# HuaiLeiTang/slam_ros

Measured on NVIDIA B200. Metric: EKF predict+update steps/s at N landmarks, higher is better.
Workload: dtype f64

## Files before the change

### slam_ros_b200/csrc/ekf_api.cu

```cuda
#include "../../include/ekf.h"
#include "ekf_internal.h"

#include <cuda.h>
#include <dlfcn.h>
#include <math.h>
#include <stdio.h>
#include <stdlib.h>
#include <string.h>
#include <vector>

namespace {
typedef struct ncclComm* ncclComm_t;
typedef struct { char internal[128]; } ncclUniqueId;
struct NcclApi {
  void* handle;
  int (*GetUniqueId)(ncclUniqueId*);
  int (*CommInitRank)(ncclComm_t*, int, ncclUniqueId, int);
  int (*CommDestroy)(ncclComm_t);
  int (*AllReduce)(const void*, void*, size_t, int, int, ncclComm_t, cudaStream_t);
  const char* (*GetErrorString)(int);
};
const int kNcclFloat64 = 8, kNcclSum = 0;

NcclApi* nccl_api() {
// ... 72 lines not shown
  double* xchg;
  void* peer_map[8];
  EkfPeers peers;
  int peers_mapped;
  int peers_ok;
  int poisoned;
  double* d_stage; size_t stage_elems;
  double* d_partials; double* d_out3;
  char err[256];
};

namespace {

#define CU(call)                                                                              \
  do {                                                                                        \
    cudaError_t e_ = (call);                                                                  \
    if (e_ != cudaSuccess) {                                                                  \
      snprintf(ctx->err, sizeof ctx->err, "%s:%d %.120s: %s", "ekf_api.cu", __LINE__, #call, cudaGetErrorString(e_)); \
      return EKF_ECUDA;                                                                       \
    }                                                                                         \
  } while (0)

#define NOT_POISONED(ctx)                                                                                          \
  do {                                                                                                             \
    if ((ctx)->poisoned) {                                                                                         \
      snprintf((ctx)->err, sizeof (ctx)->err, "a cross-GPU exchange timed out earlier (EKF_ENCCL): re-upload the state with ekf_upload"); \
      return EKF_ESTATE;                                                                                           \
    }                                                                                                              \
  } while (0)

const size_t kStageElems = (size_t)8 << 20;
const int kOverlapMinN = 6000;
static int line_sms_env() { static int v = -2; if (v == -2) { const char* e = getenv("EKF_LINE_SMS"); v = e ? atoi(e) : -1; if (v < 1 || v > 64) v = -1; } return v; }
static int line_sms_for(int world, int cap, int m) {
  const int e = line_sms_env();
  if (e > 0) return e;
  if (world >= 4) return 28;
  const int need = (cap + 511) / 512;
  return (world == 1 && m > 8 && need > 20 && need <= 28) ? need : 20;
}

double* in_u(ekf_ctx* c) { return c->d_in; }
double* in_x(ekf_ctx* c) { return c->d_in + 3; }
double* in_z(ekf_ctx* c) { return c->d_in + 6; }
double* in_R(ekf_ctx* c) { return c->d_in + 6 + 2 * (size_t)c->max_lines; }

void use_tables(ekf_ctx* ctx, int t) {
  ctx->b.jbest = ctx->tab[t].jbest; ctx->b.jout = ctx->tab[t].jout; ctx->b.pidx = ctx->tab[t].pidx;
  ctx->b.eidx = ctx->tab[t].eidx; ctx->b.ext = ctx->tab[t].ext; ctx->b.ext_cs = ctx->tab[t].ext_cs;
}

int free_line_tables(ekf_ctx* ctx) {
  for (int t = 0; t < 2; ++t) {
    cudaFree(ctx->tab[t].jbest); cudaFree(ctx->tab[t].jout); cudaFree(ctx->tab[t].pidx); cudaFree(ctx->tab[t].eidx);
    cudaFree(ctx->tab[t].ext); cudaFree(ctx->tab[t].ext_cs);
    memset(&ctx->tab[t], 0, sizeof ctx->tab[t]);
  }
  cudaFree(ctx->d_in);
  cudaFreeHost(ctx->h_in); cudaFreeHost(ctx->h_jout);
  ctx->b.jbest = ctx->b.jout = ctx->b.pidx = ctx->b.eidx = ctx->b.ext = 0; ctx->b.ext_cs = 0; ctx->d_in = 0;
  ctx->h_in = 0; ctx->h_jout = 0;
  return 0;
}

int drain(ekf_ctx* ctx);
int close_group(ekf_ctx* ctx);

int ensure_lines(ekf_ctx* ctx, int m) {
  if (m <= ctx->max_lines) return EKF_OK;
  if (ctx->scan_open && ctx->cursor > 0) {
    snprintf(ctx->err, sizeof ctx->err, "scan has more than %d lines; raise it by calling ekf_scan once with m lines", ctx->max_lines);
    return EKF_EINVAL;
// ... 176 lines not shown
  cudaEvent_t e0 = 0, e1 = 0;
  if (ctx->prof) {
    if (ctx->ev_used + 2 > ctx->ev.size())
      for (int i = 0; i < 64; ++i) { cudaEvent_t e; CU(cudaEventCreate(&e)); ctx->ev.push_back(e); }
    e0 = ctx->ev[ctx->ev_used]; e1 = ctx->ev[ctx->ev_used + 1];
    CU(cudaEventRecord(e0, ctx->wstream));
  }
  CU(ekf_launch_sweep_tma(ctx->g, bt, &ctx->tmap2[tgt], ctx->have_tmap8 ? &ctx->tmap8[tgt] : 0, &ctx->tmapK[0], &ctx->tmapK[1], ctx->Pbuf[tgt ^ 1], slot0, &ctx->d_view[par], ctx->d_counters + 16,
                          ctx->sweep_shape, nterms, L_ub, ctx->num_sms - line_sms, ctx->wstream,
                          &ctx->tmap2[tgt ^ 1], ctx->have_tmap8 ? &ctx->tmap8[tgt ^ 1] : 0));
  { const int per_pass = ekf_sweep_terms_per_pass(ctx->sweep_shape, nterms); ctx->launches += (nterms + per_pass - 1) / per_pass; }
  if (ctx->prof) {
    CU(cudaEventRecord(e1, ctx->wstream));
    ctx->ev_used += 2;
    ctx->ev_bytes.push_back((double)nterms);
  }
  CU(cudaEventRecord(ctx->evF[par], ctx->wstream));
  ctx->evF_used[par] = 1;
  ctx->rd = tgt; ctx->pg_valid = 1; ctx->pg_slot0 = slot0;
  ctx->par ^= 1;
  ctx->b.P = ctx->Pbuf[ctx->rd];
  return EKF_OK;
}

int close_group(ekf_ctx* ctx) {
  if (!ctx->grp_open) return EKF_OK;
  ctx->grp_open = 0;
  return hand_off_sweep(ctx, ctx->grp_terms, ctx->L_ub, ctx->grp_line_sms);
}

int enqueue_scan_overlapped(ekf_ctx* ctx, const double* d_u, const double* d_x_t0, int m, const double* d_z, const double* d_R) {
  const bool chunked = ctx->chunk_lines > 0 && m > ctx->chunk_above && ctx->g.world == 1;
  const int chunk = chunked ? ctx->chunk_lines : m;
  const int line_sms = line_sms_for(ctx->g.world, ctx->g.cap, m);
  const bool groupable = ctx->grp_budget > 0 && !chunked && ctx->g.world == 1;
  const bool joins = groupable && ctx->grp_open && ctx->grp_terms + m <= ctx->grp_budget && line_sms == ctx->grp_line_sms;
  if (!joins) { int rc = close_group(ctx); if (rc) return rc; }
  const int grp_terms = joins ? ctx->grp_terms + m : m;
  const bool stays_open = groupable && grp_terms + m <= ctx->grp_budget;
  if (line_sms > ctx->last_line_sms && ctx->pg_valid && ctx->evF_used[ctx->par ^ 1])
    CU(cudaStreamWaitEvent(ctx->stream, ctx->evF[ctx->par ^ 1], 0));
  ctx->last_line_sms = line_sms;
  use_tables(ctx, ctx->tabpar);
  ctx->tabpar ^= 1;
  long long lub = (long long)ctx->L_ub + m;
  const int L_after_ub = (int)(lub > ctx->g.cap ? ctx->g.cap : lub);
  { int rc = line_event(ctx); if (rc) return rc; }
  for (int line0 = 0; line0 < m; line0 += chunk) {
    const int line1 = line0 + chunk < m ? line0 + chunk : m;
    const bool first = line0 == 0, last = line1 == m;
    const int par = ctx->par;
    if (ctx->evF_used[par]) CU(cudaStreamWaitEvent(ctx->stream, ctx->evF[par], 0));
    const int slot0 = par * ctx->group;
    EkfBuffers b = ctx->b;
    b.P = ctx->Pbuf[ctx->rd];
    const int* carry = joins ? &ctx->d_view[par].cnt : 0;
    const bool fuse = first && ekf_scan_lines_fuses_predict(ctx->peers_ok ? &ctx->peers : 0) && !ctx->no_fuse;
    if (first && !fuse) { CU(ekf_launch_predict(ctx->g, b, d_u, d_x_t0, m, ctx->L_ub, ctx->stream, carry)); ctx->launches++; }
    CU(ekf_launch_scan_lines(ctx->g, b, d_z, d_R, line0, line1, line_sms, 1, slot0, ctx->pg_slot0,
                             ctx->pg_valid ? &ctx->d_view[par ^ 1].cnt : 0, ctx->peers_ok ? &ctx->peers : 0, ctx->L_ub, ctx->stream,
                             fuse ? d_u : 0, fuse ? d_x_t0 : 0, m, fuse ? carry : 0));
    ctx->launches++;
    const int tgt = ctx->pg_valid ? (ctx->rd ^ 1) : ctx->rd;
    EkfBuffers bt = ctx->b;
    bt.P = ctx->Pbuf[tgt];
    if (last) {
      if (joins && ctx->grp_may_reset && ctx->pg_valid && ctx->evF_used[par ^ 1])
// ... 823 lines not shown
```

### slam_ros_b200/csrc/ekf_internal.h

```cpp
#ifndef EKF_INTERNAL_H
#define EKF_INTERNAL_H

#include <cuda_runtime.h>
#include <limits.h>

#define EKF_TILE 64
#define EKF_LD_ALIGN 256
#define EKF_NO_MATCH INT_MAX
#define EKF_STICKY_CAPACITY 1
#define EKF_STICKY_SINGULAR 2
#define EKF_STICKY_XCHG 4

struct EkfDevState {
  double pose[3];
  double x_pre[3];
  double v[2];
  double S[4];
  int L;
  int epoch;
  int sticky;
  int n_added;
  int resets;
  int pbase;
  int np;
  int xseq;
  int L0;
};

struct EkfScanView { int cnt; int L; int pad[2]; };

struct EkfPeers { double* xchg[8]; int world, rank; };

struct EkfGeom {
  int cap;
  int n;
  int ld;
  int rank, world;
  double gate, enc_noise;
  int headroom;
  double gate_d2max;
};

struct EkfBuffers {
  EkfDevState* st;
  double* y;
  double* top;
  double* diag;
  double* P;
  int* matched;
  double2* Kp;
  double2* KSp;
  double* gates;
  double* colA;
  double* colB;
  int* jbest;
  int* jout;
  int* pidx;
  int* eidx;
  int* ext;
// ... 60 lines not shown
```

### slam_ros_b200/csrc/ekf_kernels.cu

```cuda
#include "ekf_internal.h"
#include "ekf_device.cuh"
#include <stdlib.h>
#include <string.h>
#include <cuda.h>
#include <cooperative_groups.h>
namespace cg = cooperative_groups;

#define EKF_BLOCK 256

namespace {

__device__ __forceinline__ int owner_of_row(const EkfGeom& g, int r) { return (r / EKF_TILE) % g.world; }
__device__ __forceinline__ size_t local_row(const EkfGeom& g, int r) {
  return (size_t)((r / EKF_TILE) / g.world) * EKF_TILE + (size_t)(r % EKF_TILE);
}
__device__ __forceinline__ bool is_hot(int r, int q) {
  return r <= 2 || q == r || (q == r + 1 && (r & 1));
}
__device__ __forceinline__ double hot_value(const EkfGeom& g, const EkfBuffers& b, int r, int q) {
  if (r <= 2) return b.top[(size_t)r * g.ld + q];
  const int j = (r - 3) >> 1;
  if (r & 1) return b.diag[4 * j + (q - r)];
  return b.diag[4 * j + 2];
}
// ... 318 lines not shown
      for (int t = 0; t < 8; ++t) if (i0 + t < npt) {
        d.pa = sub_rank2(d.pa, d.v[t], s_ka[i0 + t]);
        d.pb = sub_rank2(d.pb, d.v[t], s_kb[i0 + t]);
      }
    }
  } else if (d.kind == 2) {
    for (int i0 = 0; i0 < npt; i0 += 8) {
      if (i0 > 0) {
#pragma unroll
        for (int t = 0; t < 8; ++t) if (i0 + t < npt) d.v[t] = b.Kp[(size_t)pl.slot(i0 + t) * g.ld + r];
      }
#pragma unroll
      for (int t = 0; t < 8; ++t) if (i0 + t < npt) {
        d.pa = sub_rank2(d.pa, s_ksa[i0 + t], d.v[t]);
        d.pb = sub_rank2(d.pb, s_ksb[i0 + t], d.v[t]);
      }
    }
  }
}
__device__ __forceinline__ void gain_row_emit(const EkfGeom& g, const EkfBuffers& b, const Gate& G, int r, int out_slot,
                                              const GainRow& d) {
  double2 Kr, KSr;
  gain_row(G, d.p0, d.p1, d.p2, d.pa, d.pb, Kr, KSr);
  b.Kp[(size_t)out_slot * g.ld + r] = Kr;
  b.KSp[(size_t)out_slot * g.ld + r] = KSr;
}

__device__ __forceinline__ double* xchg_col(const EkfPeers& pe, const EkfGeom& g, int p, int par, int which) {
  return pe.xchg[p] + ((size_t)(2 * par + which)) * g.ld;
}
__device__ __forceinline__ unsigned long long* xchg_flags(const EkfPeers& pe, const EkfGeom& g, int p) {
  return reinterpret_cast<unsigned long long*>(pe.xchg[p] + (size_t)4 * g.ld);
}
__device__ __forceinline__ unsigned long long ld_acquire_sys(const unsigned long long* p) {
  unsigned long long v;
  asm volatile("ld.acquire.sys.global.u64 %0, [%1];" : "=l"(v) : "l"(p) : "memory");
  return v;
}
__device__ __forceinline__ void st_relaxed_sys(unsigned long long* p, unsigned long long v) {
  asm volatile("st.relaxed.sys.global.u64 [%0], %1;" ::"l"(p), "l"(v) : "memory");
}
__device__ __forceinline__ void xgpu_exchange_barrier(const EkfPeers& pe, const EkfGeom& g, unsigned long long epoch, int* sticky) {
  __threadfence_system();
  for (int p = 0; p < pe.world; ++p) st_relaxed_sys(xchg_flags(pe, g, p) + pe.rank, epoch);
  const unsigned long long* mine = xchg_flags(pe, g, pe.rank);
  for (int q = 0; q < pe.world; ++q) {
    long long spins = 0;
    while (ld_acquire_sys(mine + q) < epoch) {
      if (++spins > 40000000LL) { atomicOr(sticky, EKF_STICKY_XCHG); break; }
    }
  }
}

#ifdef EKF_LINE_TIMING
__device__ unsigned long long g_line_ts[64 * 16];
__device__ __forceinline__ unsigned long long gtimer() { unsigned long long t; asm volatile("mov.u64 %0, %%globaltimer;" : "=l"(t)); return t; }
#define TS(slot) do { if (gtid == 0 && line - line0 < 64) g_line_ts[(line - line0) * 16 + (slot)] = gtimer(); } while (0)
#else
#define TS(slot) do { } while (0)
#endif

template <int FL_THREADS, bool COOP, bool SHARD>
__global__ void __launch_bounds__(FL_THREADS, FL_THREADS == 256 ? 3 : 1) k_scan_lines(EkfGeom g, EkfBuffers b, const double* __restrict__ z,
                                                              const double* __restrict__ R, int line0, int line1,
                                                              int own_slot0, int prev_slot0, const int* __restrict__ prev_cnt_ptr,
                                                              EkfPeers pe) {
  __shared__ int s_min[FL_THREADS / 32];
  __shared__ double2 s_ka[FL_MAXP], s_kb[FL_MAXP], s_ksa[FL_MAXP], s_ksb[FL_MAXP];
  const int prev_cnt = prev_cnt_ptr ? *prev_cnt_ptr : 0;
  EkfDevState* st = b.st;
  const int gtid = blockIdx.x * blockDim.x + threadIdx.x;
  const int gstride = gridDim.x * blockDim.x;
  auto group_sync = [] () {
    if (COOP) cg::this_grid().sync(); else cg::this_cluster().sync();
  };
  const int L = st->L, nl = 3 + 2 * L, epoch = st->epoch, pbase = st->pbase;
  int nm = b.pidx[line0];
  int ne = b.eidx[line0];
  const int xseq0 = SHARD ? st->xseq : 0;
  int xdone = 0;
  double A[3][3], xp[3];
  load_rr(g, b.top, A);
  xp[0] = st->x_pre[0]; xp[1] = st->x_pre[1]; xp[2] = st->x_pre[2];
  bool have_prev = false;
  int np_prev = 0;
  double pv0 = 0.0, pv1 = 0.0;
  double pS[4] = {0, 0, 0, 0};
  for (int line = line0; line <= line1; ++line) {
    const bool gating = line < line1;
    if (!gating && !have_prev) break;
    TS(0);
    double Rl[4] = {0, 0, 0, 0}, z0 = 0, z1 = 0;
// ... 171 lines not shown
    nm += 1;
    pv0 = G.v[0]; pv1 = G.v[1];
    for (int t = 0; t < 4; ++t) pS[t] = G.S[t];
  }
  if (SHARD && gtid == 0) st->xseq = xseq0 + xdone;
}

struct HotLm { double t0a, t0b, t1a, t1b, t2a, t2b, daa, dab, dbb, ya, yb; int mt; };
__device__ __forceinline__ void hot_load(const EkfGeom& g, const EkfBuffers& b, int j, HotLm& h) {
  const int a = 3 + 2 * j;
  h.t0a = b.top[a]; h.t0b = b.top[a + 1];
  h.t1a = b.top[(size_t)g.ld + a]; h.t1b = b.top[(size_t)g.ld + a + 1];
  h.t2a = b.top[(size_t)2 * g.ld + a]; h.t2b = b.top[(size_t)2 * g.ld + a + 1];
  h.daa = b.diag[4 * j]; h.dab = b.diag[4 * j + 1]; h.dbb = b.diag[4 * j + 2];
  h.ya = b.y[a]; h.yb = b.y[a + 1];
  h.mt = b.matched[j];
}
__device__ __forceinline__ void hot_store(const EkfGeom& g, const EkfBuffers& b, int j, const HotLm& h) {
  const int a = 3 + 2 * j;
  b.top[a] = h.t0a; b.top[a + 1] = h.t0b;
  b.top[(size_t)g.ld + a] = h.t1a; b.top[(size_t)g.ld + a + 1] = h.t1b;
  b.top[(size_t)2 * g.ld + a] = h.t2a; b.top[(size_t)2 * g.ld + a + 1] = h.t2b;
  b.diag[4 * j] = h.daa; b.diag[4 * j + 1] = h.dab; b.diag[4 * j + 2] = h.dbb;
  b.y[a] = h.ya; b.y[a + 1] = h.yb;
}

template <int FL_THREADS, bool COOP, bool CACHED>
__global__ void __launch_bounds__(FL_THREADS, 1) k_scan_lines2(EkfGeom g, EkfBuffers b, const double* __restrict__ z,
                                                               const double* __restrict__ R, int line0, int line1,
                                                               int own_slot0, int prev_slot0, const int* __restrict__ prev_cnt_ptr,
                                                               const double* __restrict__ pred_u, const double* __restrict__ pred_x, int pred_m,
                                                               const int* __restrict__ pred_carry) {
  __shared__ int s_min[FL_THREADS / 32];
  __shared__ double2 s_ka[FL_MAXP], s_kb[FL_MAXP], s_ksa[FL_MAXP], s_ksb[FL_MAXP];
  const int prev_cnt = prev_cnt_ptr ? *prev_cnt_ptr : 0;
  EkfDevState* st = b.st;
  const int gtid = blockIdx.x * blockDim.x + threadIdx.x;
  const int gstride = gridDim.x * blockDim.x;
  const int scribe = gstride - 1;
  auto group_sync = [] () {
    if (COOP) cg::this_grid().sync(); else cg::this_cluster().sync();
  };
  if (pred_u) {
    predict_body(g, b, pred_u, pred_x, pred_m, gtid, gstride, pred_carry);
    __threadfence();
    group_sync();
  }
  const int L = st->L, epoch = st->epoch, pbase = st->pbase;
  int nm = b.pidx[line0];
  int ne = b.eidx[line0];
  double A[3][3], xp[3];
  load_rr(g, b.top, A);
  xp[0] = st->x_pre[0]; xp[1] = st->x_pre[1]; xp[2] = st->x_pre[2];
  constexpr bool cached = CACHED;
  HotLm h;
  if (cached && gtid < L) hot_load(g, b, gtid, h);
  PendingList pl;
  pl.prev_cnt = prev_cnt; pl.prev_slot0 = prev_slot0; pl.own_slot0 = own_slot0;
  for (int line = line0; line < line1; ++line) {
    TS(0);
    const double Rl[4] = {R[4 * line], R[4 * line + 1], R[4 * line + 2], R[4 * line + 3]};
    const double z0 = z[2 * line], z1 = z[2 * line + 1];
    int cand = EKF_NO_MATCH;
    for (int j = gtid; j < L; j += gstride) {
      if (!cached) hot_load(g, b, j, h);
      if (cand == EKF_NO_MATCH && h.mt != epoch) {
        double Cm[5][5];
        for (int r = 0; r < 3; ++r) for (int q = 0; q < 3; ++q) Cm[r][q] = A[r][q];
        Cm[0][3] = Cm[3][0] = h.t0a; Cm[0][4] = Cm[4][0] = h.t0b;
        Cm[1][3] = Cm[3][1] = h.t1a; Cm[1][4] = Cm[4][1] = h.t1b;
        Cm[2][3] = Cm[3][2] = h.t2a; Cm[2][4] = Cm[4][2] = h.t2b;
        Cm[3][3] = h.daa; Cm[3][4] = Cm[4][3] = h.dab; Cm[4][4] = h.dbb;
        Gate G;
        gate_from_block(Cm, h.ya, h.yb, xp, z0, z1, Rl, G);
        if (G.singular) atomicOr(&st->sticky, EKF_STICKY_SINGULAR);
        else if (!gate_rejects_d2(G.d2, g.gate_d2max)) {
          cand = j;
          double* rec = b.gates + (size_t)GATE_REC * j;
          gate_store(rec, G);
          rec[14] = h.t0a; rec[15] = h.t0b; rec[16] = h.t1a; rec[17] = h.t1b; rec[18] = h.t2a; rec[19] = h.t2b;
        }
      }
    }
    TS(1);
    cand = __reduce_min_sync(0xffffffffu, cand);
    if ((threadIdx.x & 31) == 0) s_min[threadIdx.x >> 5] = cand;
    __syncthreads();
    if (threadIdx.x < 32) {
      int v = (threadIdx.x < FL_THREADS / 32) ? s_min[threadIdx.x] : EKF_NO_MATCH;
      v = __reduce_min_sync(0xffffffffu, v);
      if (threadIdx.x == 0 && v != EKF_NO_MATCH) atomicMin(&b.jbest[line], v);
    }
    TS(2);
    group_sync();
    TS(3);
    const int jw = b.jbest[line];
    const int np = nm - pbase;
    if (jw != EKF_NO_MATCH) TS(8);
    if (jw == EKF_NO_MATCH) {
      if (gtid == scribe) { b.ext[ne] = line; b.eidx[line + 1] = ne + 1; b.pidx[line + 1] = nm; b.jout[line] = -1; }
      ne += 1;
      continue;
    }
    const int aw = 3 + 2 * jw, bw = aw + 1;
    const double* rec = b.gates + (size_t)GATE_REC * jw;
    Gate G;
    gate_load(rec, G);
    TS(9);
    const double wt[3][2] = {{rec[14], rec[15]}, {rec[16], rec[17]}, {rec[18], rec[19]}};
    const int npt = prev_cnt + np;
    for (int i = threadIdx.x; i < npt; i += blockDim.x) {
      const int slot = pl.slot(i);
      s_ka[i] = b.Kp[(size_t)slot * g.ld + aw]; s_kb[i] = b.Kp[(size_t)slot * g.ld + bw];
      s_ksa[i] = b.KSp[(size_t)slot * g.ld + aw]; s_ksb[i] = b.KSp[(size_t)slot * g.ld + bw];
    }
    const int out_slot = own_slot0 + np;
    double2 kk[3], ks[3];
#pragma unroll
    for (int r = 0; r < 3; ++r) gain_row(G, A[r][0], A[r][1], A[r][2], wt[r][0], wt[r][1], kk[r], ks[r]);
    if (gtid == scribe) {
#pragma unroll
      for (int r = 0; r < 3; ++r) { b.Kp[(size_t)out_slot * g.ld + r] = kk[r]; b.KSp[(size_t)out_slot * g.ld + r] = ks[r]; }
    }
    TS(10);
    const double v0 = G.v[0], v1 = G.v[1];
    constexpr int CH = 4;
    const int jc = gtid;
    const bool own1 = cached && jc < L;
    double cpa[2] = {0.0, 0.0}, cpb[2] = {0.0, 0.0};
    double2 cv[2][CH];
    int ckind = 0;
    if (own1 && jc != jw) {
      const int a = 3 + 2 * jc;
      ckind = jc < jw ? 1 : 2;
#pragma unroll
      for (int hf = 0; hf < 2; ++hf) {
        const int r = a + hf;
        if (ckind == 1) { cpa[hf] = b.P[(size_t)r * g.ld + aw]; cpb[hf] = b.P[(size_t)r * g.ld + bw]; }
        else { cpa[hf] = b.P[(size_t)aw * g.ld + r]; cpb[hf] = b.P[(size_t)bw * g.ld + r]; }
        const double2* src = ckind == 1 ? b.KSp : b.Kp;
#pragma unroll
        for (int t = 0; t < CH; ++t) if (t < npt) cv[hf][t] = src[(size_t)pl.slot(t) * g.ld + r];
      }
    }
    TS(11);
    __syncthreads();
    TS(4);
    for (int j = gtid; j < L; j += gstride) {
      const int a = 3 + 2 * j, bb = a + 1;
      double2 Ka, KSa, Kb, KSb;
      if (cached) {
        double pa0 = cpa[0], pb0 = cpb[0], pa1 = cpa[1], pb1 = cpb[1];
        if (j == jw) { pa0 = h.daa; pb0 = h.dab; pa1 = h.dab; pb1 = h.dbb; }
        else {
          const double2* src = ckind == 1 ? b.KSp : b.Kp;
          for (int i0 = 0; i0 < npt; i0 += CH) {
            if (i0 > 0) {
#pragma unroll
              for (int t = 0; t < CH; ++t) if (i0 + t < npt) {
                cv[0][t] = src[(size_t)pl.slot(i0 + t) * g.ld + a]; cv[1][t] = src[(size_t)pl.slot(i0 + t) * g.ld + bb];
              }
            }
#pragma unroll
            for (int t = 0; t < CH; ++t) if (i0 + t < npt) {
              if (ckind == 1) {
                pa0 = sub_rank2(pa0, cv[0][t], s_ka[i0 + t]); pb0 = sub_rank2(pb0, cv[0][t], s_kb[i0 + t]);
                pa1 = sub_rank2(pa1, cv[1][t], s_ka[i0 + t]); pb1 = sub_rank2(pb1, cv[1][t], s_kb[i0 + t]);
              } else {
                pa0 = sub_rank2(pa0, s_ksa[i0 + t], cv[0][t]); pb0 = sub_rank2(pb0, s_ksb[i0 + t], cv[0][t]);
                pa1 = sub_rank2(pa1, s_ksa[i0 + t], cv[1][t]); pb1 = sub_rank2(pb1, s_ksb[i0 + t], cv[1][t]);
              }
            }
          }
        }
        TS(12);
        gain_row(G, h.t0a, h.t1a, h.t2a, pa0, pb0, Ka, KSa);
        gain_row(G, h.t0b, h.t1b, h.t2b, pa1, pb1, Kb, KSb);
      } else {
        hot_load(g, b, j, h);
#pragma unroll
        for (int half = 0; half < 2; ++half) {
          const int r = a + half;
          GainRow d;
          d.p0 = half ? h.t0b : h.t0a; d.p1 = half ? h.t1b : h.t1a; d.p2 = half ? h.t2b : h.t2a;
          d.kind = 0;
          if (j == jw) { d.pa = half ? h.dab : h.daa; d.pb = half ? h.dbb : h.dab; }
          else if (j < jw) {
            const double* Pr = b.P + (size_t)r * g.ld;
            d.pa = Pr[aw]; d.pb = Pr[bw];
            d.kind = 1;
#pragma unroll
            for (int t = 0; t < 8; ++t) if (t < npt) d.v[t] = b.KSp[(size_t)pl.slot(t) * g.ld + r];
          } else {
            d.pa = b.P[(size_t)aw * g.ld + r]; d.pb = b.P[(size_t)bw * g.ld + r];
            d.kind = 2;
#pragma unroll
            for (int t = 0; t < 8; ++t) if (t < npt) d.v[t] = b.Kp[(size_t)pl.slot(t) * g.ld + r];
          }
          gain_row_correct(g, b, r, npt, d, pl, s_ka, s_kb, s_ksa, s_ksb);
          if (half) gain_row(G, d.p0, d.p1, d.p2, d.pa, d.pb, Kb, KSb);
          else gain_row(G, d.p0, d.p1, d.p2, d.pa, d.pb, Ka, KSa);
        }
      }
      TS(13);
      b.Kp[(size_t)out_slot * g.ld + a] = Ka; b.KSp[(size_t)out_slot * g.ld + a] = KSa;
      b.Kp[(size_t)out_slot * g.ld + bb] = Kb; b.KSp[(size_t)out_slot * g.ld + bb] = KSb;
      h.t0a = sub_rank2(h.t0a, ks[0], Ka); h.t0b = sub_rank2(h.t0b, ks[0], Kb);
      h.t1a = sub_rank2(h.t1a, ks[1], Ka); h.t1b = sub_rank2(h.t1b, ks[1], Kb);
      h.t2a = sub_rank2(h.t2a, ks[2], Ka); h.t2b = sub_rank2(h.t2b, ks[2], Kb);
      h.daa = sub_rank2(h.daa, KSa, Ka); h.dab = sub_rank2(h.dab, KSa, Kb); h.dbb = sub_rank2(h.dbb, KSb, Kb);
      double ta = 0.0, tb = 0.0;
      axpy_skip(ta, Ka.x, v0); axpy_skip(ta, Ka.y, v1);
      axpy_skip(tb, Kb.x, v0); axpy_skip(tb, Kb.y, v1);
      h.ya = add_rn(h.ya, ta); h.yb = add_rn(h.yb, tb);
      if (j == jw) { h.mt = epoch; b.matched[j] = epoch; }
      hot_store(g, b, j, h);
    }
    TS(5);
    update_robot_block(kk, ks, v0, v1, A, xp);
    if (gtid == scribe) {
      for (int r = 0; r < 3; ++r) {
        for (int q = r; q < 3; ++q) b.top[(size_t)r * g.ld + q] = A[r][q];
        b.y[r] = xp[r]; st->pose[r] = xp[r]; st->x_pre[r] = xp[r];
      }
      st->v[0] = v0; st->v[1] = v1;
      for (int t = 0; t < 4; ++t) st->S[t] = G.S[t];
      b.jout[line] = jw;
      b.pidx[line + 1] = nm + 1; b.eidx[line + 1] = ne;
      st->np = np + 1;
    }
    TS(6);
    nm += 1;
  }
}

__global__ void k_flush_done(EkfBuffers b, int next_line) {
  if (blockIdx.x == 0 && threadIdx.x == 0) { b.st->pbase = b.pidx[next_line]; b.st->np = 0; }
}

__global__ void k_chunk_mark(EkfBuffers b, int next_line, EkfScanView* view) {
  if (blockIdx.x == 0 && threadIdx.x == 0) {
    EkfDevState* st = b.st;
    view->cnt = b.pidx[next_line] - st->pbase; view->L = st->L;
    st->pbase = b.pidx[next_line]; st->np = 0;
  }
}

__global__ void k_queue_all(EkfGeom g, EkfBuffers b, int m) {
  const int gid = blockIdx.x * blockDim.x + threadIdx.x;
  for (int i = gid; i < m; i += gridDim.x * blockDim.x) {
    b.ext[i] = i; b.eidx[i + 1] = i + 1; b.pidx[i + 1] = 0; b.jout[i] = -1;
  }
}

struct TileId { int k, rb, cb; };

__device__ __forceinline__ long long tiles_before(int T, int rank, int world, long long k) {
  return k * (long long)(T - rank) - (long long)world * k * (k - 1) / 2;
}
__device__ __forceinline__ TileId decode_tile(int T, int rank, int world, long long idx) {
  const double A = (double)(T - rank) + 0.5 * world;
  double disc = A * A - 2.0 * world * (double)idx;
  if (disc < 0.0) disc = 0.0;
  long long k = (long long)((A - sqrt(disc)) / world);
  if (k < 0) k = 0;
  while (tiles_before(T, rank, world, k + 1) <= idx) ++k;
// ... 453 lines not shown
      for (int mb = 0; mb < 2; ++mb)
#pragma unroll
        for (int nb = 0; nb < 8; ++nb) dmma884(acc[mb][nb].x, acc[mb][nb].y, a[mb], bq[nb]);
    }
    __syncwarp();
    if (lane == 0) mbar_arrive(&sh.empty[s]);
    double* Pt = dst + ((size_t)lrow0 + row0) * g.ld + (size_t)col0 + 2 * tq;
    if (grow0 + TR <= nl && col0 + TC <= nl) {
#pragma unroll
      for (int mb = 0; mb < 2; ++mb)
#pragma unroll
        for (int nb = 0; nb < 8; ++nb) __stcs(reinterpret_cast<double2*>(Pt + (size_t)(8 * mb) * g.ld + 8 * nb), acc[mb][nb]);
    } else {
#pragma unroll
      for (int mb = 0; mb < 2; ++mb) {
        if (grow0 + row0 + 8 * mb < nl) {
          double* Pr = Pt + (size_t)(8 * mb) * g.ld;
#pragma unroll
          for (int nb = 0; nb < 8; ++nb) {
            const int q = col0 + 8 * nb + 2 * tq;
            if (q + 1 < nl) __stcs(reinterpret_cast<double2*>(Pr + 8 * nb), acc[mb][nb]); else if (q < nl) Pr[8 * nb] = acc[mb][nb].x;
          }
        }
      }
    }
  }
}

__global__ void __launch_bounds__(512) k_end_scan_a(EkfGeom g, EkfBuffers b, const double* __restrict__ z, const double* __restrict__ R, int m,
                                                    int slot0, EkfScanView* view, int prev_slot0, const int* __restrict__ prev_cnt_ptr) {
  EkfDevState* st = b.st;
  __shared__ double s_pose[3];
  __shared__ double s_y01[2];
  if (threadIdx.x == 0) {
    if (m == 0 || b.pidx[m] == 0) {
      b.y[0] = st->x_pre[0]; b.y[1] = st->x_pre[1]; b.y[2] = st->x_pre[2];
      double th = st->x_pre[2];
      normalize_radian(th);
      st->pose[0] = st->x_pre[0]; st->pose[1] = st->x_pre[1]; st->pose[2] = th;
    }
    s_pose[0] = st->pose[0]; s_pose[1] = st->pose[1]; s_pose[2] = st->pose[2];
    s_y01[0] = b.y[0]; s_y01[1] = b.y[1];
  }
  __syncthreads();
  const int ne = b.eidx[m];
  const int L = st->L;
  const int n_add = min(ne, g.cap - L);
  if (threadIdx.x == 0 && blockIdx.x == 0) {
    st->n_added = n_add;
    if (n_add < ne) atomicOr(&st->sticky, EKF_STICKY_CAPACITY);
  }
  {
    const int cnt = b.pidx[m] - st->pbase, r0 = 3 + 2 * L, r1 = 3 + 2 * (L + n_add);
    const int pcnt = prev_cnt_ptr ? *prev_cnt_ptr : 0;
    for (int i = 0; i < cnt + pcnt; ++i) {
      const size_t slot = i < cnt ? slot0 + i : prev_slot0 + (i - cnt);
      for (int r = r0 + threadIdx.x; r < r1; r += blockDim.x) {
        b.Kp[slot * g.ld + r] = make_double2(0.0, 0.0);
        b.KSp[slot * g.ld + r] = make_double2(0.0, 0.0);
      }
    }
  }
  double A[3][3];
  load_rr(g, b.top, A);
  for (int e = blockIdx.x * blockDim.x + threadIdx.x; e < n_add; e += gridDim.x * blockDim.x) {
    const int i = b.ext[e];
// ... 24 lines not shown
      }
    double GR[2][2] = {{0, 0}, {0, 0}};
    for (int k = 0; k < 2; ++k)
      for (int ii = 0; ii < 2; ++ii) {
        const double t = mul_rn(1.0, Gl[ii][k]);
        if (t != 0.0) for (int jj = 0; jj < 2; ++jj) GR[ii][jj] = add_rn(GR[ii][jj], mul_rn(t, Rl[k * 2 + jj]));
      }
    for (int ii = 0; ii < 2; ++ii)
      for (int jj = 0; jj < 2; ++jj) {
        double t = 0.0;
        for (int k = 0; k < 2; ++k) t = add_rn(t, mul_rn(GR[ii][k], Gl[jj][k]));
        Pll[ii][jj] = add_rn(Pll[ii][jj], add_rn(0.0, mul_rn(1.0, t)));
      }
    b.diag[4 * (L + e)] = Pll[0][0]; b.diag[4 * (L + e) + 1] = Pll[0][1]; b.diag[4 * (L + e) + 2] = Pll[1][1];
    b.diag[4 * (L + e) + 3] = 0.0;
    for (int k = 0; k < 3; ++k) {
      double r0 = 0.0, r1 = 0.0;
      for (int kk = 0; kk < 3; ++kk) {
        axpy_skip(r0, mul_rn(1.0, Gx[0][kk]), A[kk][k]);
        axpy_skip(r1, mul_rn(1.0, Gx[1][kk]), A[kk][k]);
      }
      b.top[(size_t)k * g.ld + l] = r0;
      b.top[(size_t)k * g.ld + l + 1] = r1;
    }
  }
  __syncthreads();
  if (threadIdx.x == 0) {
    st->L0 = L;
    int Ln = L + n_add;
    const bool reset = Ln > g.cap - g.headroom;
    if (reset) { Ln = 0; st->resets += 1; }
    st->L = Ln;
    if (view) { view->cnt = reset ? 0 : b.pidx[m] - st->pbase; view->L = Ln; }
  }
}

__global__ void __launch_bounds__(EKF_BLOCK) k_end_scan_b(EkfGeom g, EkfBuffers b, double* __restrict__ P2) {
  const EkfDevState* st = b.st;
  const int n_add = st->n_added;
  const int L = st->L0;
  const int c_idx = blockIdx.x * blockDim.x + threadIdx.x;
  if (c_idx >= 2 * n_add) return;
  const int e = c_idx >> 1, tsel = c_idx & 1;
  const int l = 3 + 2 * (L + e);
  const int col = l + tsel;
  const double cw = b.ext_cs[2 * e], sw = b.ext_cs[2 * e + 1];
  const double* t0p = b.top; const double* t1p = b.top + g.ld; const double* t2p = b.top + 2 * (size_t)g.ld;
  for (int k = 3 + blockIdx.y; k < l; k += gridDim.y) {
    if (g.world > 1 && owner_of_row(g, k) != g.rank) continue;
    double v;
    if (tsel == 0) { v = 0.0; axpy_skip(v, 1.0, t2p[k]); }
    else { v = 0.0; axpy_skip(v, cw, t0p[k]); axpy_skip(v, sw, t1p[k]); }
    b.P[local_row(g, k) * g.ld + col] = v;
    if (P2) P2[local_row(g, k) * g.ld + col] = v;
  }
}

__global__ void __launch_bounds__(EKF_BLOCK) k_assemble(EkfGeom g, EkfBuffers b, int r0, int nr, int c0, int nc,
                                                        double* __restrict__ out, int ld_out) {
  const int nl = 3 + 2 * b.st->L;
  const long long total = (long long)nr * nc;
  for (long long t = blockIdx.x * (long long)blockDim.x + threadIdx.x; t < total;
       t += (long long)gridDim.x * blockDim.x) {
    const int r = r0 + (int)(t / nc), q = c0 + (int)(t % nc);
    double v = 0.0;
    if (r < nl && q < nl) {
      const int lo = min(r, q), hi = max(r, q);
      if (is_hot(lo, hi)) { if (g.rank == 0) v = hot_value(g, b, lo, hi); }
      else if (g.world == 1 || owner_of_row(g, lo) == g.rank) v = b.P[local_row(g, lo) * g.ld + hi];
    }
    out[(size_t)(r - r0) * ld_out + (q - c0)] = v;
  }
}

__global__ void __launch_bounds__(EKF_BLOCK) k_scatter(EkfGeom g, EkfBuffers b, int r0, int nr, int nl,
                                                       const double* __restrict__ in, int ld_in) {
  const long long total = (long long)nr * nl;
  for (long long t = blockIdx.x * (long long)blockDim.x + threadIdx.x; t < total;
       t += (long long)gridDim.x * blockDim.x) {
    const int r = r0 + (int)(t / nl), q = (int)(t % nl);
    if (q < r) continue;
    const double v = in[(size_t)(r - r0) * ld_in + q];
    if (r <= 2) b.top[(size_t)r * g.ld + q] = v;
    else if (is_hot(r, q)) {
      const int j = (r - 3) >> 1;
      if (r & 1) b.diag[4 * j + (q - r)] = v; else b.diag[4 * j + 2] = v;
    } else if (g.world == 1 || owner_of_row(g, r) == g.rank) b.P[local_row(g, r) * g.ld + q] = v;
  }
// ... 50 lines not shown
}

}

cudaError_t ekf_launch_init(const EkfGeom& g, const EkfBuffers& b, cudaStream_t s) {
  k_init<<<1, 32, 0, s>>>(g, b);
  return cudaGetLastError();
}
cudaError_t ekf_launch_predict(const EkfGeom& g, const EkfBuffers& b, const double* d_u, const double* d_x_t0,
                               int m, int L_ub, cudaStream_t s, const int* carry) {
  const int work = (3 + 2 * L_ub > m) ? 3 + 2 * L_ub : m;
  k_predict<<<blocks_for(work, 1024), EKF_BLOCK, 0, s>>>(g, b, d_u, d_x_t0, m, carry);
  return cudaGetLastError();
}
cudaError_t ekf_launch_associate(const EkfGeom& g, const EkfBuffers& b, const double* d_z, const double* d_R,
                                 int line, int L_ub, cudaStream_t s) {
  if (L_ub <= 0) return cudaSuccess;
  k_associate<<<blocks_for(L_ub), EKF_BLOCK, 0, s>>>(g, b, d_z, d_R, line);
  return cudaGetLastError();
}
cudaError_t ekf_launch_gain(const EkfGeom& g, const EkfBuffers& b, const double* d_z, const double* d_R,
                            int line, int j_override, int mode, int L_ub, int max_batch, cudaStream_t s) {
  if (L_ub <= 0) return cudaSuccess;
  k_gain<<<blocks_for(3 + 2 * L_ub, 2048), EKF_BLOCK, 0, s>>>(g, b, d_z, d_R, line, j_override, mode, max_batch);
  return cudaGetLastError();
}
cudaError_t ekf_launch_apply(const EkfGeom& g, const EkfBuffers& b, int line, int j_override, int L_ub,
                             cudaStream_t s) {
  k_apply<<<blocks_for(3 + 2 * L_ub, 2048), EKF_BLOCK, 0, s>>>(g, b, line, j_override);
  return cudaGetLastError();
}
#ifdef EKF_LINE_TIMING
extern "C" int ekf_debug_line_timing(unsigned long long* out, int n) {
  return (int)cudaMemcpyFromSymbol(out, g_line_ts, sizeof(unsigned long long) * (size_t)n);
}
#endif
void ekf_prefer_max_smem_carveout(void) {
  const int c = cudaSharedmemCarveoutMaxShared;
  cudaFuncSetAttribute(k_predict, cudaFuncAttributePreferredSharedMemoryCarveout, c);
  cudaFuncSetAttribute(k_scan_lines<512, true, false>, cudaFuncAttributePreferredSharedMemoryCarveout, c);
  cudaFuncSetAttribute(k_scan_lines<512, true, true>, cudaFuncAttributePreferredSharedMemoryCarveout, c);
  cudaFuncSetAttribute(k_scan_lines<512, false, false>, cudaFuncAttributePreferredSharedMemoryCarveout, c);
  cudaFuncSetAttribute(k_scan_lines2<512, true, true>, cudaFuncAttributePreferredSharedMemoryCarveout, c);
  cudaFuncSetAttribute(k_scan_lines2<512, true, false>, cudaFuncAttributePreferredSharedMemoryCarveout, c);
  cudaFuncSetAttribute(k_scan_lines2<512, false, true>, cudaFuncAttributePreferredSharedMemoryCarveout, c);
  cudaFuncSetAttribute(k_scan_lines2<256, false, true>, cudaFuncAttributePreferredSharedMemoryCarveout, c);
  cudaFuncSetAttribute(k_scan_lines2<512, false, false>, cudaFuncAttributePreferredSharedMemoryCarveout, c);
  cudaFuncSetAttribute(k_end_scan_a, cudaFuncAttributePreferredSharedMemoryCarveout, c);
  cudaFuncSetAttribute(k_end_scan_b, cudaFuncAttributePreferredSharedMemoryCarveout, c);
  cudaFuncSetAttribute(k_chunk_mark, cudaFuncAttributePreferredSharedMemoryCarveout, c);
  cudaFuncSetAttribute(k_queue_all, cudaFuncAttributePreferredSharedMemoryCarveout, c);
  (void)cudaGetLastError();
}
static int line_loop_v1() { static int v = -1; if (v < 0) { const char* e = getenv("EKF_LINE_LOOP"); v = (e && atoi(e) == 1) ? 1 : 0; } return v; }
int ekf_pick_cluster(void) {
  cudaFuncSetAttribute(k_scan_lines<512, false, false>, cudaFuncAttributeNonPortableClusterSizeAllowed, 1);
  cudaFuncSetAttribute(k_scan_lines2<512, false, true>, cudaFuncAttributeNonPortableClusterSizeAllowed, 1);
  cudaFuncSetAttribute(k_scan_lines2<256, false, true>, cudaFuncAttributeNonPortableClusterSizeAllowed, 1);
  cudaFuncSetAttribute(k_scan_lines2<512, false, false>, cudaFuncAttributeNonPortableClusterSizeAllowed, 1);
  { const char* e = getenv("EKF_CLUSTER"); const int v = e ? atoi(e) : 0; if (v == 1 || v == 2 || v == 4 || v == 8) return v; }
  const int tries[2] = {16, 8};
  for (int t = 0; t < 2; ++t) {
    cudaLaunchConfig_t cfg;
    memset(&cfg, 0, sizeof cfg);
    cfg.gridDim = dim3(tries[t]); cfg.blockDim = dim3(512);
    cudaLaunchAttribute attr[1];
    attr[0].id = cudaLaunchAttributeClusterDimension;
    attr[0].val.clusterDim.x = tries[t]; attr[0].val.clusterDim.y = 1; attr[0].val.clusterDim.z = 1;
    cfg.attrs = attr; cfg.numAttrs = 1;
    int n = 0;
    int n2 = 0;
    if (cudaOccupancyMaxActiveClusters(&n, k_scan_lines<512, false, false>, &cfg) == cudaSuccess && n >= 1 &&
        cudaOccupancyMaxActiveClusters(&n2, k_scan_lines2<512, false, false>, &cfg) == cudaSuccess && n2 >= 1) return tries[t];
  }
  (void)cudaGetLastError();
  return 8;
}
int ekf_scan_lines_fuses_predict(const EkfPeers* peers) { return !line_loop_v1() && !(peers && peers->world > 1); }
cudaError_t ekf_launch_scan_lines(const EkfGeom& g, const EkfBuffers& b, const double* d_z, const double* d_R,
                                  int line0, int line1, int ctas, int coop, int own_slot0, int prev_slot0,
                                  const int* prev_cnt_ptr, const EkfPeers* peers, int L_ub, cudaStream_t s,
                                  const double* pred_u, const double* pred_x, int pred_m, const int* pred_carry) {
  if (line1 <= line0) return cudaSuccess;
  if (pred_u && !ekf_scan_lines_fuses_predict(peers)) return cudaErrorInvalidValue;
  EkfPeers pe;
  memset(&pe, 0, sizeof pe);
  pe.world = 1;
  if (peers) pe = *peers;
  if (coop) {
    void* args[] = {(void*)&g, (void*)&b, (void*)&d_z, (void*)&d_R, (void*)&line0, (void*)&line1, (void*)&own_slot0,
                    (void*)&prev_slot0, (void*)&prev_cnt_ptr, (void*)&pe};
    if (peers && peers->world > 1)
      return cudaLaunchCooperativeKernel((const void*)k_scan_lines<512, true, true>, dim3(ctas), dim3(512), args, 0, s);
    if (line_loop_v1())
      return cudaLaunchCooperativeKernel((const void*)k_scan_lines<512, true, false>, dim3(ctas), dim3(512), args, 0, s);
    void* args2[] = {(void*)&g, (void*)&b, (void*)&d_z, (void*)&d_R, (void*)&line0, (void*)&line1, (void*)&own_slot0,
                     (void*)&prev_slot0, (void*)&prev_cnt_ptr, (void*)&pred_u, (void*)&pred_x, (void*)&pred_m, (void*)&pred_carry};
    static int lt = -1;
    if (lt < 0) { const char* e = getenv("EKF_LINE_THREADS"); lt = e ? atoi(e) : 0; }
    if (L_ub > g.cap) L_ub = g.cap;
    if (lt == 256 && L_ub <= ctas * 256)
      return cudaLaunchCooperativeKernel((const void*)k_scan_lines2<256, true, true>, dim3(ctas), dim3(256), args2, 0, s);
    if (L_ub <= ctas * 512) return cudaLaunchCooperativeKernel((const void*)k_scan_lines2<512, true, true>, dim3(ctas), dim3(512), args2, 0, s);
    return cudaLaunchCooperativeKernel((const void*)k_scan_lines2<512, true, false>, dim3(ctas), dim3(512), args2, 0, s);
  }
  cudaLaunchConfig_t cfg;
  memset(&cfg, 0, sizeof cfg);
  cfg.gridDim = dim3(ctas); cfg.blockDim = dim3(512); cfg.dynamicSmemBytes = 0; cfg.stream = s;
  cudaLaunchAttribute attr[1];
  attr[0].id = cudaLaunchAttributeClusterDimension;
  attr[0].val.clusterDim.x = ctas; attr[0].val.clusterDim.y = 1; attr[0].val.clusterDim.z = 1;
  cfg.attrs = attr; cfg.numAttrs = 1;
  if (line_loop_v1())
    return cudaLaunchKernelEx(&cfg, k_scan_lines<512, false, false>, g, b, d_z, d_R, line0, line1, own_slot0, prev_slot0, prev_cnt_ptr, pe);
  if (L_ub <= ctas * 256) {
    cfg.blockDim = dim3(256);
    return cudaLaunchKernelEx(&cfg, k_scan_lines2<256, false, true>, g, b, d_z, d_R, line0, line1, own_slot0, prev_slot0, prev_cnt_ptr, pred_u, pred_x, pred_m, pred_carry);
  }
  if (L_ub <= ctas * 512)
    return cudaLaunchKernelEx(&cfg, k_scan_lines2<512, false, true>, g, b, d_z, d_R, line0, line1, own_slot0, prev_slot0, prev_cnt_ptr, pred_u, pred_x, pred_m, pred_carry);
  return cudaLaunchKernelEx(&cfg, k_scan_lines2<512, false, false>, g, b, d_z, d_R, line0, line1, own_slot0, prev_slot0, prev_cnt_ptr, pred_u, pred_x, pred_m, pred_carry);
}
cudaError_t ekf_launch_flush_done(const EkfBuffers& b, int next_line, cudaStream_t s) {
  k_flush_done<<<1, 32, 0, s>>>(b, next_line);
  return cudaGetLastError();
}
cudaError_t ekf_launch_chunk_mark(const EkfBuffers& b, int next_line, EkfScanView* view, cudaStream_t s) {
  k_chunk_mark<<<1, 32, 0, s>>>(b, next_line, view);
  return cudaGetLastError();
}
cudaError_t ekf_launch_queue_all(const EkfGeom& g, const EkfBuffers& b, int m, cudaStream_t s) {
  if (m <= 0) return cudaSuccess;
  k_queue_all<<<blocks_for(m, 1024), EKF_BLOCK, 0, s>>>(g, b, m);
// ... 211 lines not shown
```

Measured before the change: 3174.

## Replace per-line grid sync with flag-based all-to-all min exchange in cooperative line scan

In the cooperative line-scan kernel, the per-line grid.sync plus atomicMin on jbest is replaced by a tagged release/acquire slot array. Each CTA publishes its local minimum to that array and spins until every other CTA's entry is present. The rank-2 downdate of the cached columns is also moved ahead of the gain computation so it does not depend on the winning gate record, and the line-SMS heuristic no longer depends on m. This targets the latency of a full grid barrier per line, at the cost of spin-polling global memory and a new cap of 64 CTAs. Extended timing instrumentation is added under a debug macro.

```diff
diff --git a/slam_ros_b200/csrc/ekf_api.cu b/slam_ros_b200/csrc/ekf_api.cu
--- a/slam_ros_b200/csrc/ekf_api.cu
+++ b/slam_ros_b200/csrc/ekf_api.cu
@@ -128,12 +128,12 @@
 const size_t kStageElems = (size_t)8 << 20;
 const int kOverlapMinN = 6000;
 static int line_sms_env() { static int v = -2; if (v == -2) { const char* e = getenv("EKF_LINE_SMS"); v = e ? atoi(e) : -1; if (v < 1 || v > 64) v = -1; } return v; }
-static int line_sms_for(int world, int cap, int m) {
+static int line_sms_for(int world, int cap) {
   const int e = line_sms_env();
   if (e > 0) return e;
   if (world >= 4) return 28;
   const int need = (cap + 511) / 512;
-  return (world == 1 && m > 8 && need > 20 && need <= 28) ? need : 20;
+  return (world == 1 && need > 20 && need <= 28) ? need : 20;
 }
 
 double* in_u(ekf_ctx* c) { return c->d_in; }
@@ -376,7 +376,7 @@
 int enqueue_scan_overlapped(ekf_ctx* ctx, const double* d_u, const double* d_x_t0, int m, const double* d_z, const double* d_R) {
   const bool chunked = ctx->chunk_lines > 0 && m > ctx->chunk_above && ctx->g.world == 1;
   const int chunk = chunked ? ctx->chunk_lines : m;
-  const int line_sms = line_sms_for(ctx->g.world, ctx->g.cap, m);
+  const int line_sms = line_sms_for(ctx->g.world, ctx->g.cap);
   const bool groupable = ctx->grp_budget > 0 && !chunked && ctx->g.world == 1;
   const bool joins = groupable && ctx->grp_open && ctx->grp_terms + m <= ctx->grp_budget && line_sms == ctx->grp_line_sms;
   if (!joins) { int rc = close_group(ctx); if (rc) return rc; }
diff --git a/slam_ros_b200/csrc/ekf_internal.h b/slam_ros_b200/csrc/ekf_internal.h
--- a/slam_ros_b200/csrc/ekf_internal.h
+++ b/slam_ros_b200/csrc/ekf_internal.h
@@ -10,6 +10,7 @@
 #define EKF_STICKY_CAPACITY 1
 #define EKF_STICKY_SINGULAR 2
 #define EKF_STICKY_XCHG 4
+#define EKF_MAX_LINE_CTAS 64
 
 struct EkfDevState {
   double pose[3];
@@ -25,6 +26,8 @@
   int np;
   int xseq;
   int L0;
+  unsigned int lseq;
+  unsigned long long lslot[2][EKF_MAX_LINE_CTAS];
 };
 
 struct EkfScanView { int cnt; int L; int pad[2]; };
diff --git a/slam_ros_b200/csrc/ekf_kernels.cu b/slam_ros_b200/csrc/ekf_kernels.cu
--- a/slam_ros_b200/csrc/ekf_kernels.cu
+++ b/slam_ros_b200/csrc/ekf_kernels.cu
@@ -374,6 +374,14 @@
 __device__ __forceinline__ unsigned long long* xchg_flags(const EkfPeers& pe, const EkfGeom& g, int p) {
   return reinterpret_cast<unsigned long long*>(pe.xchg[p] + (size_t)4 * g.ld);
 }
+__device__ __forceinline__ unsigned long long ld_acquire_gpu(const unsigned long long* p) {
+  unsigned long long v;
+  asm volatile("ld.acquire.gpu.global.u64 %0, [%1];" : "=l"(v) : "l"(p) : "memory");
+  return v;
+}
+__device__ __forceinline__ void st_release_gpu(unsigned long long* p, unsigned long long v) {
+  asm volatile("st.release.gpu.global.u64 [%0], %1;" ::"l"(p), "l"(v) : "memory");
+}
 __device__ __forceinline__ unsigned long long ld_acquire_sys(const unsigned long long* p) {
   unsigned long long v;
   asm volatile("ld.acquire.sys.global.u64 %0, [%1];" : "=l"(v) : "l"(p) : "memory");
@@ -395,11 +403,21 @@
 }
 
 #ifdef EKF_LINE_TIMING
-__device__ unsigned long long g_line_ts[64 * 16];
+#define EKF_TS_SCANS 64
+#define EKF_TS_LINES 16
+#define EKF_TS_KOFF (EKF_TS_LINES * 16)
+#define EKF_TS_REC (EKF_TS_KOFF + 16)
+enum { EKF_TSK_LINES_IN = 0, EKF_TSK_PROLOGUE = 1, EKF_TSK_LINES_OUT = 2, EKF_TSK_A_IN = 3, EKF_TSK_A_OUT = 4, EKF_TSK_B_IN = 5,
+       EKF_TSK_B_OUT = 6, EKF_TSK_GROUP_POS = 7 };
+__device__ unsigned long long g_line_ts[EKF_TS_SCANS * EKF_TS_REC];
+__device__ unsigned int g_ts_scan;
 __device__ __forceinline__ unsigned long long gtimer() { unsigned long long t; asm volatile("mov.u64 %0, %%globaltimer;" : "=l"(t)); return t; }
-#define TS(slot) do { if (gtid == 0 && line - line0 < 64) g_line_ts[(line - line0) * 16 + (slot)] = gtimer(); } while (0)
+__device__ __forceinline__ unsigned long long* ts_rec(unsigned int k) { return g_line_ts + (size_t)(k % EKF_TS_SCANS) * EKF_TS_REC; }
+#define TS(slot) do { if (gtid == 0 && line < EKF_TS_LINES) ts_rec(g_ts_scan)[line * 16 + (slot)] = gtimer(); } while (0)
+#define TSK(slot) do { ts_rec(g_ts_scan)[EKF_TS_KOFF + (slot)] = gtimer(); } while (0)
 #else
 #define TS(slot) do { } while (0)
+#define TSK(slot) do { } while (0)
 #endif
 
 template <int FL_THREADS, bool COOP, bool SHARD>
@@ -637,19 +655,26 @@
                                                                const double* __restrict__ pred_u, const double* __restrict__ pred_x, int pred_m,
                                                                const int* __restrict__ pred_carry) {
   __shared__ int s_min[FL_THREADS / 32];
+  __shared__ int s_win;
+  __shared__ double s_rec[20];
   __shared__ double2 s_ka[FL_MAXP], s_kb[FL_MAXP], s_ksa[FL_MAXP], s_ksb[FL_MAXP];
   const int prev_cnt = prev_cnt_ptr ? *prev_cnt_ptr : 0;
   EkfDevState* st = b.st;
+  const unsigned int lseq0 = COOP ? st->lseq : 0u;
   const int gtid = blockIdx.x * blockDim.x + threadIdx.x;
   const int gstride = gridDim.x * blockDim.x;
   const int scribe = gstride - 1;
   auto group_sync = [] () {
     if (COOP) cg::this_grid().sync(); else cg::this_cluster().sync();
   };
+#ifdef EKF_LINE_TIMING
+  if (gtid == 0 && line0 == 0) { TSK(EKF_TSK_LINES_IN); ts_rec(g_ts_scan)[EKF_TS_KOFF + EKF_TSK_GROUP_POS] = pred_carry ? 2 : 1; }
+#endif
   if (pred_u) {
     predict_body(g, b, pred_u, pred_x, pred_m, gtid, gstride, pred_carry);
     __threadfence();
     group_sync();
+    if (gtid == 0) TSK(EKF_TSK_PROLOGUE);
   }
   const int L = st->L, epoch = st->epoch, pbase = st->pbase;
   int nm = b.pidx[line0];
@@ -691,17 +716,44 @@
     cand = __reduce_min_sync(0xffffffffu, cand);
     if ((threadIdx.x & 31) == 0) s_min[threadIdx.x >> 5] = cand;
     __syncthreads();
-    if (threadIdx.x < 32) {
-      int v = (threadIdx.x < FL_THREADS / 32) ? s_min[threadIdx.x] : EKF_NO_MATCH;
-      v = __reduce_min_sync(0xffffffffu, v);
-      if (threadIdx.x == 0 && v != EKF_NO_MATCH) atomicMin(&b.jbest[line], v);
-    }
-    TS(2);
-    group_sync();
-    TS(3);
-    const int jw = b.jbest[line];
+    int jw;
+    if (COOP) {
+      if (threadIdx.x < 32) {
+        int v = (threadIdx.x < FL_THREADS / 32) ? s_min[threadIdx.x] : EKF_NO_MATCH;
+        v = __reduce_min_sync(0xffffffffu, v);
+        const unsigned int tag = lseq0 + (unsigned int)(line - line0) + 1u;
+        unsigned long long* words = st->lslot[tag & 1u];
+        if (threadIdx.x == 0) {
+          __threadfence();
+          st_release_gpu(words + blockIdx.x, ((unsigned long long)tag << 32) | (unsigned int)v);
+        }
+        TS(2);
+        int w = EKF_NO_MATCH;
+        for (int c = threadIdx.x; c < (int)gridDim.x; c += 32) {
+          unsigned long long x;
+          do { x = ld_acquire_gpu(words + c); } while ((int)((unsigned int)(x >> 32) - tag) < 0);
+          w = min(w, (int)(unsigned int)x);
+        }
+        w = __reduce_min_sync(0xffffffffu, w);
+        if (threadIdx.x == 0) s_win = w;
+      }
+      __syncthreads();
+      jw = s_win;
+      TS(3);
+    } else {
+      if (threadIdx.x < 32) {
+        int v = (threadIdx.x < FL_THREADS / 32) ? s_min[threadIdx.x] : EKF_NO_MATCH;
+        v = __reduce_min_sync(0xffffffffu, v);
+        if (threadIdx.x == 0 && v != EKF_NO_MATCH) atomicMin(&b.jbest[line], v);
+      }
+      TS(2);
+      group_sync();
+      TS(3);
+      jw = b.jbest[line];
+    }
     const int np = nm - pbase;
     if (jw != EKF_NO_MATCH) TS(8);
+    if (COOP && gtid == scribe) b.jbest[line] = jw;
     if (jw == EKF_NO_MATCH) {
       if (gtid == scribe) { b.ext[ne] = line; b.eidx[line + 1] = ne + 1; b.pidx[line + 1] = nm; b.jout[line] = -1; }
       ne += 1;
@@ -709,10 +761,8 @@
     }
     const int aw = 3 + 2 * jw, bw = aw + 1;
     const double* rec = b.gates + (size_t)GATE_REC * jw;
-    Gate G;
-    gate_load(rec, G);
+    if (threadIdx.x < 20) s_rec[threadIdx.x] = rec[threadIdx.x];
     TS(9);
-    const double wt[3][2] = {{rec[14], rec[15]}, {rec[16], rec[17]}, {rec[18], rec[19]}};
     const int npt = prev_cnt + np;
     for (int i = threadIdx.x; i < npt; i += blockDim.x) {
       const int slot = pl.slot(i);
@@ -720,15 +770,6 @@
       s_ksa[i] = b.KSp[(size_t)slot * g.ld + aw]; s_ksb[i] = b.KSp[(size_t)slot * g.ld + bw];
     }
     const int out_slot = own_slot0 + np;
-    double2 kk[3], ks[3];
-#pragma unroll
-    for (int r = 0; r < 3; ++r) gain_row(G, A[r][0], A[r][1], A[r][2], wt[r][0], wt[r][1], kk[r], ks[r]);
-    if (gtid == scribe) {
-#pragma unroll
-      for (int r = 0; r < 3; ++r) { b.Kp[(size_t)out_slot * g.ld + r] = kk[r]; b.KSp[(size_t)out_slot * g.ld + r] = ks[r]; }
-    }
-    TS(10);
-    const double v0 = G.v[0], v1 = G.v[1];
     constexpr int CH = 4;
     const int jc = gtid;
     const bool own1 = cached && jc < L;
@@ -751,34 +792,46 @@
     TS(11);
     __syncthreads();
     TS(4);
+    double pa0 = cpa[0], pb0 = cpb[0], pa1 = cpa[1], pb1 = cpb[1];
+    if (ckind != 0) {
+      const int a = 3 + 2 * jc, bb = a + 1;
+      const double2* src = ckind == 1 ? b.KSp : b.Kp;
+      for (int i0 = 0; i0 < npt; i0 += CH) {
+        if (i0 > 0) {
+#pragma unroll
+          for (int t = 0; t < CH; ++t) if (i0 + t < npt) {
+            cv[0][t] = src[(size_t)pl.slot(i0 + t) * g.ld + a]; cv[1][t] = src[(size_t)pl.slot(i0 + t) * g.ld + bb];
+          }
+        }
+#pragma unroll
+        for (int t = 0; t < CH; ++t) if (i0 + t < npt) {
+          if (ckind == 1) {
+            pa0 = sub_rank2(pa0, cv[0][t], s_ka[i0 + t]); pb0 = sub_rank2(pb0, cv[0][t], s_kb[i0 + t]);
+            pa1 = sub_rank2(pa1, cv[1][t], s_ka[i0 + t]); pb1 = sub_rank2(pb1, cv[1][t], s_kb[i0 + t]);
+          } else {
+            pa0 = sub_rank2(pa0, s_ksa[i0 + t], cv[0][t]); pb0 = sub_rank2(pb0, s_ksb[i0 + t], cv[0][t]);
+            pa1 = sub_rank2(pa1, s_ksa[i0 + t], cv[1][t]); pb1 = sub_rank2(pb1, s_ksb[i0 + t], cv[1][t]);
+          }
+        }
+      }
+    }
+    TS(12);
+    Gate G;
+    gate_load(s_rec, G);
+    double2 kk[3], ks[3];
+#pragma unroll
+    for (int r = 0; r < 3; ++r) gain_row(G, A[r][0], A[r][1], A[r][2], s_rec[14 + 2 * r], s_rec[15 + 2 * r], kk[r], ks[r]);
+    if (gtid == scribe) {
+#pragma unroll
+      for (int r = 0; r < 3; ++r) { b.Kp[(size_t)out_slot * g.ld + r] = kk[r]; b.KSp[(size_t)out_slot * g.ld + r] = ks[r]; }
+    }
+    TS(10);
+    const double v0 = G.v[0], v1 = G.v[1];
     for (int j = gtid; j < L; j += gstride) {
       const int a = 3 + 2 * j, bb = a + 1;
       double2 Ka, KSa, Kb, KSb;
       if (cached) {
-        double pa0 = cpa[0], pb0 = cpb[0], pa1 = cpa[1], pb1 = cpb[1];
         if (j == jw) { pa0 = h.daa; pb0 = h.dab; pa1 = h.dab; pb1 = h.dbb; }
-        else {
-          const double2* src = ckind == 1 ? b.KSp : b.Kp;
-          for (int i0 = 0; i0 < npt; i0 += CH) {
-            if (i0 > 0) {
-#pragma unroll
-              for (int t = 0; t < CH; ++t) if (i0 + t < npt) {
-                cv[0][t] = src[(size_t)pl.slot(i0 + t) * g.ld + a]; cv[1][t] = src[(size_t)pl.slot(i0 + t) * g.ld + bb];
-              }
-            }
-#pragma unroll
-            for (int t = 0; t < CH; ++t) if (i0 + t < npt) {
-              if (ckind == 1) {
-                pa0 = sub_rank2(pa0, cv[0][t], s_ka[i0 + t]); pb0 = sub_rank2(pb0, cv[0][t], s_kb[i0 + t]);
-                pa1 = sub_rank2(pa1, cv[1][t], s_ka[i0 + t]); pb1 = sub_rank2(pb1, cv[1][t], s_kb[i0 + t]);
-              } else {
-                pa0 = sub_rank2(pa0, s_ksa[i0 + t], cv[0][t]); pb0 = sub_rank2(pb0, s_ksb[i0 + t], cv[0][t]);
-                pa1 = sub_rank2(pa1, s_ksa[i0 + t], cv[1][t]); pb1 = sub_rank2(pb1, s_ksb[i0 + t], cv[1][t]);
-              }
-            }
-          }
-        }
-        TS(12);
         gain_row(G, h.t0a, h.t1a, h.t2a, pa0, pb0, Ka, KSa);
         gain_row(G, h.t0b, h.t1b, h.t2b, pa1, pb1, Kb, KSb);
       } else {
@@ -837,6 +890,8 @@
     TS(6);
     nm += 1;
   }
+  if (COOP && gtid == scribe) st->lseq = lseq0 + (unsigned int)(line1 - line0);
+  if (gtid == 0) TSK(EKF_TSK_LINES_OUT);
 }
 
 __global__ void k_flush_done(EkfBuffers b, int next_line) {
@@ -1356,6 +1411,9 @@
   EkfDevState* st = b.st;
   __shared__ double s_pose[3];
   __shared__ double s_y01[2];
+#ifdef EKF_LINE_TIMING
+  if (threadIdx.x == 0) { TSK(EKF_TSK_A_IN); ts_rec(g_ts_scan)[EKF_TS_KOFF + EKF_TSK_B_OUT] = 0; }
+#endif
   if (threadIdx.x == 0) {
     if (m == 0 || b.pidx[m] == 0) {
       b.y[0] = st->x_pre[0]; b.y[1] = st->x_pre[1]; b.y[2] = st->x_pre[2];
@@ -1446,6 +1504,10 @@
     if (reset) { Ln = 0; st->resets += 1; }
     st->L = Ln;
     if (view) { view->cnt = reset ? 0 : b.pidx[m] - st->pbase; view->L = Ln; }
+#ifdef EKF_LINE_TIMING
+    TSK(EKF_TSK_A_OUT);
+    g_ts_scan += 1;
+#endif
   }
 }
 
@@ -1454,7 +1516,14 @@
   const int n_add = st->n_added;
   const int L = st->L0;
   const int c_idx = blockIdx.x * blockDim.x + threadIdx.x;
+#ifdef EKF_LINE_TIMING
+  unsigned long long* tsr = ts_rec(g_ts_scan - 1);
+  if (c_idx == 0 && blockIdx.y == 0) tsr[EKF_TS_KOFF + EKF_TSK_B_IN] = gtimer();
+  if (c_idx < 2 * n_add)
+#else
   if (c_idx >= 2 * n_add) return;
+#endif
+  {
   const int e = c_idx >> 1, tsel = c_idx & 1;
   const int l = 3 + 2 * (L + e);
   const int col = l + tsel;
@@ -1468,6 +1537,11 @@
     b.P[local_row(g, k) * g.ld + col] = v;
     if (P2) P2[local_row(g, k) * g.ld + col] = v;
   }
+  }
+#ifdef EKF_LINE_TIMING
+  __syncthreads();
+  if (threadIdx.x == 0) atomicMax(tsr + EKF_TS_KOFF + EKF_TSK_B_OUT, gtimer());
+#endif
 }
 
 __global__ void __launch_bounds__(EKF_BLOCK) k_assemble(EkfGeom g, EkfBuffers b, int r0, int nr, int c0, int nc,
@@ -1584,7 +1658,18 @@
 }
 #ifdef EKF_LINE_TIMING
 extern "C" int ekf_debug_line_timing(unsigned long long* out, int n) {
-  return (int)cudaMemcpyFromSymbol(out, g_line_ts, sizeof(unsigned long long) * (size_t)n);
+  unsigned int k = 0;
+  cudaError_t e = cudaMemcpyFromSymbol(&k, g_ts_scan, sizeof k);
+  if (e != cudaSuccess) return (int)e;
+  const size_t off = (size_t)((k + EKF_TS_SCANS - 1) % EKF_TS_SCANS) * EKF_TS_REC * sizeof(unsigned long long);
+  return (int)cudaMemcpyFromSymbol(out, g_line_ts, sizeof(unsigned long long) * (size_t)n, off);
+}
+extern "C" int ekf_debug_scan_timing(unsigned long long* out, int n) {
+  unsigned int k = 0;
+  if (n < EKF_TS_SCANS * EKF_TS_REC) return -1;
+  if (cudaMemcpyFromSymbol(&k, g_ts_scan, sizeof k) != cudaSuccess) return -1;
+  if (cudaMemcpyFromSymbol(out, g_line_ts, sizeof(unsigned long long) * EKF_TS_SCANS * EKF_TS_REC) != cudaSuccess) return -1;
+  return (int)k;
 }
 #endif
 void ekf_prefer_max_smem_carveout(void) {
@@ -1651,6 +1736,7 @@
     static int lt = -1;
     if (lt < 0) { const char* e = getenv("EKF_LINE_THREADS"); lt = e ? atoi(e) : 0; }
     if (L_ub > g.cap) L_ub = g.cap;
+    if (ctas > EKF_MAX_LINE_CTAS) return cudaErrorInvalidValue;
     if (lt == 256 && L_ub <= ctas * 256)
       return cudaLaunchCooperativeKernel((const void*)k_scan_lines2<256, true, true>, dim3(ctas), dim3(256), args2, 0, s);
     if (L_ub <= ctas * 512) return cudaLaunchCooperativeKernel((const void*)k_scan_lines2<512, true, true>, dim3(ctas), dim3(512), args2, 0, s);
```

Result: no change. 3173 (median of 6 runs) (-0.1%).
